# alpenlabs/dv-pari

Hardware: AMD Instinct MI355X
Metric: R1CS constraints/sec (prove) (higher is better)
Workload: dtype u32; 1 GPU; Proof::prove, synthetic dense R1CS, 2^20 constraints (BASELINE config #4); log2_constraints=20, n_wires=1048576, msm_pairs_per_proof=6291456, witness=resident in HBM, entry=dvp_prove_dev (Proof::prove with the witness resident), proofs_in_flight=1

## Files before the change

dv-pari_amd/csrc/msm_rounds.cuh:

```cuda
#pragma once
#include "common.h"
#include "k233.cuh"
#include "msm_scan.cuh"
#include "msm_reduce.cuh"

namespace dvp {

constexpr uint32_t AFF_NONE = 0xffffffffu;
constexpr uint32_t DESC_PAIR = 0x80000000u;

__global__ void __launch_bounds__(256)
k_post_sort(uint32_t* __restrict__ items, const uint32_t* __restrict__ cnt, const uint32_t* __restrict__ off , uint32_t nkeys,
            uint32_t* __restrict__ ocnt, uint32_t* __restrict__ ooff , uint32_t* __restrict__ d_max) {
  const uint32_t k = blockIdx.x * blockDim.x + threadIdx.x;
  uint32_t m = 0;
  if (k <= nkeys) {
    const uint32_t o = off[k];
    ooff[k] = o >> 1;
    if (k < nkeys) {
      const uint32_t c = cnt[k];
      if (c & 1) items[o + c] = AFF_NONE;
      ocnt[k] = (c + 1) >> 1;
      m = c;
    }
  }
  for (int o = 32; o > 0; o >>= 1) m = max(m, (uint32_t)__shfl_xor((int)m, o));
  if ((threadIdx.x & 63) == 0 && m) atomicMax(d_max, m);
}

__global__ void __launch_bounds__(SCAN_TPB) k_mscan_local(const uint32_t* __restrict__ cnt0, uint32_t m, int R, uint32_t* __restrict__ rp,
                                                          uint32_t* __restrict__ bs ) {
  __shared__ uint32_t sh[SCAN_TPB];
  const uint32_t base = blockIdx.x * SCAN_BLK + threadIdx.x * SCAN_EPT;
  uint32_t v[SCAN_EPT];
#pragma unroll
  for (int k = 0; k < SCAN_EPT; ++k) v[k] = (base + k < m) ? cnt0[base + k] : 0;
  {
    uint32_t mx = 0;
#pragma unroll
    for (int k = 0; k < SCAN_EPT; ++k) mx = max(mx, v[k]);
    for (int d = 32; d > 0; d >>= 1) mx = max(mx, (uint32_t)__shfl_xor((int)mx, d));
    if ((threadIdx.x & 63) == 0) sh[threadIdx.x >> 6] = mx;
    __syncthreads();
    if (threadIdx.x == 0) {
      for (int w = 1; w < SCAN_TPB / 64; ++w) mx = max(mx, sh[w]);
      bs[(size_t)R * gridDim.x + blockIdx.x] = mx;
    }
    __syncthreads();
  }
  for (int r = 1; r <= R; ++r) {
    uint32_t* c = rp + (size_t)(2 * (r - 1)) * ((size_t)m + 1);
    uint32_t* o = c + ((size_t)m + 1);
    uint32_t s = 0;
#pragma unroll
    for (int k = 0; k < SCAN_EPT; ++k) {
      v[k] = (v[k] + 1u) >> 1;
      s += v[k];
    }
    uint32_t tot;
    uint32_t ex = block_exclusive_scan(s, &tot, sh);
#pragma unroll
    for (int k = 0; k < SCAN_EPT; ++k) {
      if (base + k < m) {
        c[base + k] = v[k];
        o[base + k] = ex;
      }
      ex += v[k];
    }
    if (threadIdx.x == 0) bs[(size_t)(r - 1) * gridDim.x + blockIdx.x] = tot;
  }
}
__global__ void __launch_bounds__(SCAN_TPB) k_mscan_bsums(uint32_t* __restrict__ bs, uint32_t nb, uint32_t m, uint32_t* __restrict__ rp,
                                                          uint32_t* __restrict__ off0 ,
                                                          uint32_t* __restrict__ dmax ) {
  __shared__ uint32_t sh[SCAN_TPB];
  const int r = blockIdx.x + 1;
  uint32_t* row = bs + (size_t)(r - 1) * nb;
  uint32_t carry = 0;
  for (uint32_t base = 0; base < nb; base += SCAN_TPB) {
    uint32_t idx = base + threadIdx.x;
    uint32_t v = idx < nb ? row[idx] : 0;
    uint32_t tot;
    uint32_t ex = block_exclusive_scan(v, &tot, sh);
    if (idx < nb) row[idx] = ex + carry;
    carry += tot;
  }
  if (threadIdx.x == 0) {
    rp[(size_t)(2 * (r - 1) + 1) * ((size_t)m + 1) + m] = carry;
    if (r == 1 && off0) off0[m] = 2u * carry;
  }
  if (r == 1 && dmax) {
    const uint32_t* bm = bs + (size_t)gridDim.x * nb;
    uint32_t mx = 0;
    for (uint32_t i = threadIdx.x; i < nb; i += SCAN_TPB) mx = max(mx, bm[i]);
    for (int d = 32; d > 0; d >>= 1) mx = max(mx, (uint32_t)__shfl_xor((int)mx, d));
    __syncthreads();
    if ((threadIdx.x & 63) == 0) sh[threadIdx.x >> 6] = mx;
    __syncthreads();
    if (threadIdx.x == 0) {
      for (int w = 1; w < SCAN_TPB / 64; ++w) mx = max(mx, sh[w]);
      *dmax = mx;
    }
  }
}
__global__ void __launch_bounds__(SCAN_TPB) k_mscan_add(uint32_t* __restrict__ rp, const uint32_t* __restrict__ bs, uint32_t m, int R,
                                                        const uint32_t* __restrict__ cnt0, uint32_t* __restrict__ off0, uint32_t* __restrict__ items) {
  const uint32_t base = blockIdx.x * SCAN_BLK + threadIdx.x * SCAN_EPT;
  for (int r = 1; r <= R; ++r) {
    uint32_t* o = rp + (size_t)(2 * (r - 1) + 1) * ((size_t)m + 1);
    const uint32_t add = bs[(size_t)(r - 1) * gridDim.x + blockIdx.x];
    if (r == 1 && off0) {
#pragma unroll
      for (int k = 0; k < SCAN_EPT; ++k)
        if (base + k < m) {
          const uint32_t v = o[base + k] + add, c = cnt0[base + k];
          o[base + k] = v;
          off0[base + k] = 2u * v;
          if (c & 1u) items[2u * v + c] = AFF_NONE;
        }
      continue;
    }
#pragma unroll
    for (int k = 0; k < SCAN_EPT; ++k)
      if (base + k < m) o[base + k] += add;
  }
}
struct DescPlan {
  unsigned long long at[40];
};
template <int LPK, bool DENSE>
__global__ void __launch_bounds__(1024)
k_round_desc_all(const uint32_t* __restrict__ rp, uint32_t nkeys, int R, DescPlan plan, uint32_t* __restrict__ desc) {
  const uint32_t gid = blockIdx.x * blockDim.x + threadIdx.x;
  const uint32_t key = gid / LPK, lane = gid % LPK;
  if (key >= nkeys) return;
  const size_t stride = (size_t)nkeys + 1;
  for (int r0 = 1; r0 < R; r0 += 8) {
    uint32_t cr[8], o[8], oo[8], A[8];
#pragma unroll
    for (int q = 0; q < 8; ++q) {
      const int r = r0 + q;
      if (r < R) {
        const uint32_t* c = rp + (size_t)(2 * (r - 1)) * stride;
        cr[q] = c[key];
        o[q] = c[stride + key];
        oo[q] = c[3 * stride + key];
        A[q] = DENSE ? c[stride + nkeys] - c[3 * stride + nkeys] : 0u;
      } else {
        cr[q] = 0; o[q] = 0; oo[q] = 0; A[q] = 0;
      }
    }
#pragma unroll
    for (int q = 0; q < 8; ++q) {
      const int r = r0 + q;
      if (r >= R) break;
      const uint32_t nout = (cr[q] + 1) >> 1;
      uint32_t* d = desc + plan.at[r];
      if (DENSE) {
        const uint32_t npair = cr[q] >> 1, a = o[q] - oo[q];
        uint2* d2 = (uint2*)d;
        for (uint32_t j = lane; j < npair; j += LPK) d2[a + j] = make_uint2((o[q] + 2 * j) | DESC_PAIR, oo[q] + j);
        if ((cr[q] & 1u) && lane == npair % LPK) d2[A[q] + (2 * oo[q] - o[q])] = make_uint2(o[q] + cr[q] - 1, oo[q] + npair);
        continue;
      }
      for (uint32_t j = lane; j < nout; j += LPK) d[oo[q] + j] = (o[q] + 2 * j) | ((2 * j + 1 < cr[q]) ? DESC_PAIR : 0u);
    }
  }
}

template <int LPK>
__global__ void __launch_bounds__(256)
k_round_desc(const uint32_t* __restrict__ cnt, const uint32_t* __restrict__ off, const uint32_t* __restrict__ ooff ,
             uint32_t nkeys, uint32_t* __restrict__ desc) {
  const uint32_t gid = blockIdx.x * blockDim.x + threadIdx.x;
  const uint32_t key = gid / LPK, lane = gid % LPK;
  if (key >= nkeys) return;
  const uint32_t c = cnt[key], o = off[key], oo = ooff[key], nout = (c + 1) >> 1;
  for (uint32_t j = lane; j < nout; j += LPK) desc[oo + j] = (o + 2 * j) | ((2 * j + 1 < c) ? DESC_PAIR : 0u);
}

#ifndef AFF_PRIO
#define AFF_PRIO 1
#endif
#ifndef AFF_XY
#define AFF_XY 1
#endif
#ifndef AFF_NUM1
#define AFF_NUM1 1
#endif
__device__ __forceinline__ void aff_set_prio(uint32_t v) {
  switch (v % 3u) {
    case 0: __builtin_amdgcn_s_setprio(0); break;
    case 1: __builtin_amdgcn_s_setprio(1); break;
    default: __builtin_amdgcn_s_setprio(2); break;
  }
}
constexpr uint32_t AFF_BMAX = 136;
__device__ __forceinline__ uint32_t aff_slots_per_thread(uint32_t total, uint32_t cap, uint32_t bmax_bmin) {
  const uint32_t bmax = bmax_bmin & 0xffu, bmin = (bmax_bmin >> 8) & 0xffu;
  const uint32_t units = (total + cap - 1) / cap;
  const uint32_t R = (units + bmax - 1) / bmax;
  const uint32_t B = R ? (units + R - 1) / R : 1;
  return B < bmin ? bmin : B;
}
constexpr uint32_t AFF_SHARE_INV = 1u << 16;
constexpr uint32_t AFF_X_SLOT_BYTES = 2048;
constexpr uint32_t aff_exchange_bytes(uint32_t waves) { return waves == 4 ? 6 * AFF_X_SLOT_BYTES : waves == 2 ? 3 * AFF_X_SLOT_BYTES : 0; }
constexpr uint32_t AFF_INV_SPREAD = 256;
__device__ __forceinline__ void aff_x_put(uint32_t lane_addr, uint32_t slot, const Gf& v) {
  const uint32_t a = lane_addr + slot * AFF_X_SLOT_BYTES;
  gf_lds_st(a, (gf_u32x4){v.w[0], v.w[1], v.w[2], v.w[3]});
  gf_lds_st(a + 1024, (gf_u32x4){v.w[4], v.w[5], v.w[6], v.w[7]});
}
__device__ __forceinline__ Gf aff_x_get(uint32_t lane_addr, uint32_t slot) {
  const uint32_t a = lane_addr + slot * AFF_X_SLOT_BYTES;
  const gf_u32x4 lo = gf_lds_ld(a), hi = gf_lds_ld(a + 1024);
  Gf r;
  r.w[0] = lo.x; r.w[1] = lo.y; r.w[2] = lo.z; r.w[3] = lo.w;
  r.w[4] = hi.x; r.w[5] = hi.y; r.w[6] = hi.z; r.w[7] = hi.w;
  return r;
}
struct WaveTrace {
  unsigned long long* buf;
  uint32_t cap, tag;
};
struct AffSlot {
  uint32_t a, b, o;
};
template <bool FIRST, bool TRACE = false, bool DENSE = false>
__global__ void __launch_bounds__(EC_TPB) __attribute__((amdgpu_waves_per_eu(3, 3)))
k_affine_round(const Aff* __restrict__ pts, const uint2* __restrict__ desc, const uint32_t* __restrict__ total_ptr ,
               uint32_t cap, uint32_t bmax, GfSqrTables T, Gf* __restrict__ prefix, Aff* __restrict__ out, uint32_t sign_mask, WaveTrace wt) {
  extern __shared__ char lds_raw[];
  unsigned long long tr_t0 = 0, tr_c0 = 0, tr_t1 = 0, tr_t2 = 0;
  uint32_t tr_inverted = 0;
  if (TRACE) { tr_t0 = wall_clock64(); tr_c0 = clock64(); }
  GfLdsK L = gf_ldsk_init(lds_raw);
#if AFF_PRIO
  const uint32_t wslot = __builtin_amdgcn_s_getreg(((4 - 1) << 11) | 4);
#endif
  const uint32_t sm = FIRST ? sign_mask : 0u;
  auto ldx = [&](uint32_t v) -> Gf { return pts[v & ~sm].x; };
  auto ldy = [&](uint32_t v, const Gf& x) -> Gf {
    Gf y = pts[v & ~sm].y;
    if (v & sm) y = gf_add(y, x);
    return y;
  };
  const uint32_t total = *total_ptr;
  const int B = (int)aff_slots_per_thread(total, cap, bmax);
  const uint32_t nthr = (total + B - 1) / B;
  const uint32_t tid = blockIdx.x * blockDim.x + threadIdx.x;
  const bool share = (bmax & AFF_SHARE_INV) != 0 && blockDim.x > 64;
  if (share ? blockIdx.x * blockDim.x >= nthr : tid >= nthr) return;
  const bool wave_live = __builtin_amdgcn_readfirstlane(tid & ~63u) < nthr;
  const uint2 none = make_uint2(AFF_NONE, AFF_NONE);
  auto ld_desc = [&](int k) -> AffSlot {
    const uint32_t sk = (uint32_t)k * nthr + tid;
    const bool ok = k >= 0 && k < B && sk < total && tid < nthr;
    if (FIRST) {
      uint2 v = none;
      if (ok) v = desc[sk];
      return AffSlot{v.x, v.y, 0u};
    }
    const uint2 d = DENSE ? desc[ok ? sk : 0u] : make_uint2(((const uint32_t*)desc)[ok ? sk : 0u], 0u);
    const uint32_t a = d.x & ~DESC_PAIR;
    return AffSlot{ok ? a : AFF_NONE, (ok && (d.x & DESC_PAIR)) ? a + 1 : AFF_NONE, d.y};
  };
  const Gf one = gf_one();
  Gf run = one;
  if (wave_live) {
    AffSlot d0 = ld_desc(0), d1 = ld_desc(1);
    Gf xa = gf_zero(), xb = gf_zero();
    if (d0.b != AFF_NONE) { xa = ldx(d0.a); xb = ldx(d0.b); }
#if AFF_NUM1
    Gf ya = gf_zero(), yb = gf_zero();
    if (d0.b != AFF_NONE) { ya = ldy(d0.a, xa); yb = ldy(d0.b, xb); }
#endif
#pragma unroll 1
    for (int k = 0; k < B; ++k) {
#if AFF_PRIO
      aff_set_prio(wslot + (uint32_t)k);
#endif
      const AffSlot d2 = ld_desc(k + 2);
      Gf nxa = gf_zero(), nxb = gf_zero();
      if (d1.b != AFF_NONE) { nxa = ldx(d1.a); nxb = ldx(d1.b); }
#if AFF_NUM1
      Gf nya = gf_zero(), nyb = gf_zero();
      if (d1.b != AFF_NONE) { nya = ldy(d1.a, nxa); nyb = ldy(d1.b, nxb); }
#endif
      const bool pair = d0.b != AFF_NONE;
      if (!DENSE || __any(pair)) {
        Gf den = one;
#if AFF_NUM1
        Gf num = gf_zero();
        if (pair && !gf_is_zero(xa) && !gf_is_zero(xb)) {
          const Gf dd = gf_add(xa, xb), ys = gf_add(ya, yb);
          if (!gf_is_zero(dd)) { den = dd; num = ys; }
          else if (gf_is_zero(ys)) { den = xa; num = ya; }
        }
        Gf np, nrun;
        gf_mul2(num, den, run, L, np, nrun);
        if (pair) prefix[(size_t)k * nthr + tid] = np;
        run = nrun;
#else
        if (pair && !gf_is_zero(xa) && !gf_is_zero(xb)) {
          Gf dd = gf_add(xa, xb);
          if (!gf_is_zero(dd)) den = dd;
          else if (gf_eq(ldy(d0.a, xa), ldy(d0.b, xb))) den = xa;
        }
        if (pair) prefix[(size_t)k * nthr + tid] = run;
        run = gf_mul(run, den, L);
#endif
      }
      d0 = d1; d1 = d2; xa = nxa; xb = nxb;
#if AFF_NUM1
      ya = nya; yb = nyb;
#endif
    }
  }
  if (TRACE) tr_t1 = wall_clock64();
  const uint32_t W = blockDim.x >> 6, w = __builtin_amdgcn_readfirstlane(threadIdx.x >> 6);
  const uint32_t xa = L.lane_base + (W - w) * GF_LDSK_BYTES_PER_WAVE;
  const uint32_t inverting = (blockIdx.x / AFF_INV_SPREAD) & (W - 1);
  Gf inv = run;
  if (share) {
    if (TRACE) tr_inverted = w == inverting ? 3u : 2u;
    aff_x_put(xa, w, run);
    __syncthreads();
    if (W == 4) {
      if ((w & 1u) == 0) aff_x_put(xa, 4 + (w >> 1), gf_mul(run, aff_x_get(xa, w + 1), L));
      __syncthreads();
    }
    if (w == inverting) {
      __builtin_amdgcn_s_setprio(3);
      inv = gf_mul(aff_x_get(xa, W == 4 ? 4 : 0), aff_x_get(xa, W == 4 ? 5 : 1), L);
    }
  }
  if (!share || w == inverting) inv = gf_inv_fast(inv, T, L);
  if (share) {
    if (w == inverting) {
      if (W == 4) {
        Gf ia, ib;
        gf_mul2(aff_x_get(xa, 5), aff_x_get(xa, 4), inv, L, ia, ib);
        aff_x_put(xa, 4, ia);
        aff_x_put(xa, 5, ib);
      } else {
        aff_x_put(xa, 2, inv);
      }
      __builtin_amdgcn_s_setprio(0);
    }
    __syncthreads();
    inv = gf_mul(aff_x_get(xa, W == 4 ? 4 + (w >> 1) : 2), aff_x_get(xa, w ^ 1u), L);
  }
  if (TRACE) tr_t2 = wall_clock64();
  if (wave_live) {
    AffSlot e0 = ld_desc(B - 1), e1 = ld_desc(B - 2);
    Gf px = gf_zero(), qx = gf_zero(), pre = one;
    if (e0.a != AFF_NONE) px = ldx(e0.a);
    if (e0.b != AFF_NONE) { qx = ldx(e0.b); pre = prefix[(size_t)(B - 1) * nthr + tid]; }
#if AFF_XY
    Gf py = gf_zero();
    if (e0.a != AFF_NONE) py = ldy(e0.a, px);
#if !AFF_NUM1
    Gf qy = gf_zero();
    if (e0.b != AFF_NONE) qy = ldy(e0.b, qx);
#endif
#endif
#pragma unroll 1
    for (int k = B - 1; k >= 0; --k) {
#if AFF_PRIO
      aff_set_prio(wslot + (uint32_t)k);
#endif
      const AffSlot e2 = ld_desc(k - 2);
#if AFF_XY
      Gf npx = gf_zero(), nqx = gf_zero(), npy = gf_zero(), npre = one;
      if (e1.a != AFF_NONE) { npx = ldx(e1.a); npy = ldy(e1.a, npx); }
#if AFF_NUM1
      if (e1.b != AFF_NONE) { nqx = ldx(e1.b); npre = prefix[(size_t)(k - 1) * nthr + tid]; }
#else
      Gf nqy = gf_zero();
      if (e1.b != AFF_NONE) { nqx = ldx(e1.b); nqy = ldy(e1.b, nqx); npre = prefix[(size_t)(k - 1) * nthr + tid]; }
#endif
#else
      Gf py = gf_zero();
      if (e0.a != AFF_NONE) py = ldy(e0.a, px);
#if !AFF_NUM1
      Gf qy = gf_zero();
      if (e0.b != AFF_NONE) qy = ldy(e0.b, qx);
#endif
      Gf npx = gf_zero(), nqx = gf_zero(), npre = one;
      if (e1.a != AFF_NONE) npx = ldx(e1.a);
      if (e1.b != AFF_NONE) { nqx = ldx(e1.b); npre = prefix[(size_t)(k - 1) * nthr + tid]; }
#endif
#if AFF_NUM1
      auto q_y = [&]() -> Gf { return ldy(e0.b, qx); };
#else
      auto q_y = [&]() -> Gf { return qy; };
#endif
      if (e0.a != AFF_NONE) {
        const uint32_t sidx = DENSE ? e0.o : (uint32_t)k * nthr + tid;
        Gf ox = px, oy = py;
        if (e0.b != AFF_NONE) {
          if (gf_is_zero(px)) { ox = qx; oy = q_y(); }
          else if (!gf_is_zero(qx)) {
            Gf dd = gf_add(px, qx);
            const bool same_x = gf_is_zero(dd);
            const bool dbl = same_x && gf_eq(py, q_y());
            if (same_x && !dbl) {
              ox = gf_zero(); oy = gf_zero();
            } else {
              Gf den = dbl ? px : dd;
#if AFF_NUM1
              Gf lam, inv_next;
              gf_mul2(pre, den, inv, L, lam, inv_next);
              inv = inv_next;
#else
              Gf dinv, inv_next;
              gf_mul2(pre, den, inv, L, dinv, inv_next);
              inv = inv_next;
              Gf num = dbl ? py : gf_add(py, qy);
              Gf lam = gf_mul(num, dinv, L);
#endif
              if (dbl) lam = gf_add(lam, px);
              ox = gf_add(gf_add(gf_sqr(lam), lam), dd);
              oy = gf_add(gf_add(gf_mul(gf_add(px, ox), lam, L), ox), py);
            }
          }
        }
        out[sidx].x = ox; out[sidx].y = oy;
      }
      e0 = e1; e1 = e2; px = npx; qx = nqx; pre = npre;
#if AFF_XY
      py = npy;
#if !AFF_NUM1
      qy = nqy;
#endif
#endif
    }
  }
#if AFF_PRIO
  __builtin_amdgcn_s_setprio(0);
#endif
  if (TRACE) {
    const unsigned long long t3 = wall_clock64(), c3 = clock64();
    if ((threadIdx.x & 63u) == 0) {
      const unsigned long long i = atomicAdd(wt.buf, 1ull);
      if (i < wt.cap) {
        unsigned long long* r = wt.buf + 8 + 8 * i;
        r[0] = tr_t0; r[1] = tr_t1; r[2] = tr_t2; r[3] = t3;
        r[4] = tr_c0; r[5] = c3;
        r[6] = (unsigned long long)__builtin_amdgcn_s_getreg((31 << 11) | 4) | ((unsigned long long)__builtin_amdgcn_s_getreg((31 << 11) | 20) << 32);
        r[7] = (unsigned long long)blockIdx.x | ((unsigned long long)wt.tag << 32) | ((unsigned long long)(uint32_t)B << 48) | ((unsigned long long)(threadIdx.x >> 6) << 56) |
               ((unsigned long long)tr_inverted << 60);
      }
    }
  }
}

__global__ void __launch_bounds__(256)
k_bucket_gather_aff(const Aff* __restrict__ in, const uint32_t* __restrict__ cnt, const uint32_t* __restrict__ off,
                    uint32_t nkeys, Ld* __restrict__ A) {
  uint32_t k = blockIdx.x * blockDim.x + threadIdx.x;
  if (k >= nkeys) return;
  Ld r = ld_infinity();
  if (cnt[k]) {
    Aff p = in[off[k]];
    if (!gf_is_zero(p.x)) r = ld_from_aff(p);
  }
  A[k] = r;
}
__global__ void __launch_bounds__(256)
k_bucket_gather_items(const Aff* __restrict__ bases, const uint32_t* __restrict__ items, const uint32_t* __restrict__ cnt,
                      const uint32_t* __restrict__ off, uint32_t nkeys, Ld* __restrict__ A, uint32_t sign_mask) {
  uint32_t k = blockIdx.x * blockDim.x + threadIdx.x;
  if (k >= nkeys) return;
  Ld r = ld_infinity();
  if (cnt[k]) {
    const uint32_t v = items[off[k]];
    Aff q = bases[v & ~sign_mask];
    if (v & sign_mask) q.y = gf_add(q.y, q.x);
    r = ld_from_aff(q);
  }
  A[k] = r;
}

__global__ void __launch_bounds__(256)
k_bucket_gather(const Ld* __restrict__ in, const uint32_t* __restrict__ cnt, const uint32_t* __restrict__ off,
                uint32_t nkeys, Ld* __restrict__ A) {
  uint32_t k = blockIdx.x * blockDim.x + threadIdx.x;
  if (k >= nkeys) return;
  A[k] = cnt[k] ? in[off[k]] : ld_infinity();
}

}
```

Measured before the change: 59.17 million constraints/s.

## Flag rare affine-add cases in prefix words and load points branch-free

Rewrites the batched-affine addition kernel so the forward pass computes den and num unconditionally. It detects infinity, same-x and doubling cases with OR-reduction, and encodes the rare outcome in spare high bits of the stored prefix product. The backward pass reads those flags instead of re-checking zero/equality and reloading q's y, and only leaves the common add path when a flag is set. Point and descriptor loads become unconditional (index 0 when absent), the sign fix-up becomes a mask-xor, and slot indices advance by addition instead of multiplication. The intent is to cut divergent branches, redundant y loads and extra comparisons. In exchange it issues extra loads for empty slots and depends on the top bits of word 7 being unused by K-233 field elements.

```diff
diff --git a/dv-pari_amd/csrc/msm_rounds.cuh b/dv-pari_amd/csrc/msm_rounds.cuh
--- a/dv-pari_amd/csrc/msm_rounds.cuh
+++ b/dv-pari_amd/csrc/msm_rounds.cuh
@@ -182,12 +182,10 @@
 #ifndef AFF_PRIO
 #define AFF_PRIO 1
 #endif
-#ifndef AFF_XY
-#define AFF_XY 1
-#endif
-#ifndef AFF_NUM1
-#define AFF_NUM1 1
-#endif
+constexpr uint32_t AFF_W7_MASK = 0x1ffu, AFF_W7_DBL = 1u << 30, AFF_W7_SKIP = 1u << 31;
+__device__ __forceinline__ uint32_t aff_or8(const Gf& a) {
+  return ((a.w[0] | a.w[1] | a.w[2]) | (a.w[3] | a.w[4])) | ((a.w[5] | a.w[6]) | a.w[7]);
+}
 __device__ __forceinline__ void aff_set_prio(uint32_t v) {
   switch (v % 3u) {
     case 0: __builtin_amdgcn_s_setprio(0); break;
@@ -227,6 +225,26 @@
 struct AffSlot {
   uint32_t a, b, o;
 };
+template <bool FIRST>
+__device__ __forceinline__ void aff_ld_point(const Aff* __restrict__ pts, uint32_t sm, uint32_t v, Gf& x, Gf& y) {
+  const Aff* p = pts + (v & ~sm);
+  x = p->x;
+  y = p->y;
+  if (FIRST) {
+    const uint32_t neg = 0u - (uint32_t)((v & sm) != 0u);
+#pragma unroll
+    for (int i = 0; i < 8; ++i) y.w[i] = gf_andxor(neg, x.w[i], y.w[i]);
+  }
+}
+template <bool FIRST, bool DENSE>
+__device__ __forceinline__ AffSlot aff_ld_desc(const uint2* __restrict__ desc, int k, int B, uint32_t sk, uint32_t lim) {
+  const bool ok = k >= 0 && k < B && sk < lim;
+  const uint32_t at = ok ? sk : 0u;
+  const uint2 d = (FIRST || DENSE) ? desc[at] : make_uint2(((const uint32_t*)desc)[at], 0u);
+  if (FIRST) return AffSlot{ok ? d.x : AFF_NONE, ok ? d.y : AFF_NONE, 0u};
+  const uint32_t a = d.x & ~DESC_PAIR;
+  return AffSlot{ok ? a : AFF_NONE, (ok && (d.x & DESC_PAIR)) ? a + 1 : AFF_NONE, d.y};
+}
 template <bool FIRST, bool TRACE = false, bool DENSE = false>
 __global__ void __launch_bounds__(EC_TPB) __attribute__((amdgpu_waves_per_eu(3, 3)))
 k_affine_round(const Aff* __restrict__ pts, const uint2* __restrict__ desc, const uint32_t* __restrict__ total_ptr ,
@@ -241,11 +259,7 @@
 #endif
   const uint32_t sm = FIRST ? sign_mask : 0u;
   auto ldx = [&](uint32_t v) -> Gf { return pts[v & ~sm].x; };
-  auto ldy = [&](uint32_t v, const Gf& x) -> Gf {
-    Gf y = pts[v & ~sm].y;
-    if (v & sm) y = gf_add(y, x);
-    return y;
-  };
+  auto ldp = [&](uint32_t v, Gf& x, Gf& y) { aff_ld_point<FIRST>(pts, sm, v, x, y); };
   const uint32_t total = *total_ptr;
   const int B = (int)aff_slots_per_thread(total, cap, bmax);
   const uint32_t nthr = (total + B - 1) / B;
@@ -253,69 +267,61 @@
   const bool share = (bmax & AFF_SHARE_INV) != 0 && blockDim.x > 64;
   if (share ? blockIdx.x * blockDim.x >= nthr : tid >= nthr) return;
   const bool wave_live = __builtin_amdgcn_readfirstlane(tid & ~63u) < nthr;
-  const uint2 none = make_uint2(AFF_NONE, AFF_NONE);
-  auto ld_desc = [&](int k) -> AffSlot {
-    const uint32_t sk = (uint32_t)k * nthr + tid;
-    const bool ok = k >= 0 && k < B && sk < total && tid < nthr;
-    if (FIRST) {
-      uint2 v = none;
-      if (ok) v = desc[sk];
-      return AffSlot{v.x, v.y, 0u};
-    }
-    const uint2 d = DENSE ? desc[ok ? sk : 0u] : make_uint2(((const uint32_t*)desc)[ok ? sk : 0u], 0u);
-    const uint32_t a = d.x & ~DESC_PAIR;
-    return AffSlot{ok ? a : AFF_NONE, (ok && (d.x & DESC_PAIR)) ? a + 1 : AFF_NONE, d.y};
-  };
+  const uint32_t lim = tid < nthr ? total : 0u;
+  auto ld_desc = [&](int k, uint32_t sk) -> AffSlot { return aff_ld_desc<FIRST, DENSE>(desc, k, B, sk, lim); };
   const Gf one = gf_one();
   Gf run = one;
   if (wave_live) {
-    AffSlot d0 = ld_desc(0), d1 = ld_desc(1);
-    Gf xa = gf_zero(), xb = gf_zero();
-    if (d0.b != AFF_NONE) { xa = ldx(d0.a); xb = ldx(d0.b); }
-#if AFF_NUM1
-    Gf ya = gf_zero(), yb = gf_zero();
-    if (d0.b != AFF_NONE) { ya = ldy(d0.a, xa); yb = ldy(d0.b, xb); }
-#endif
+    uint32_t sk = tid, sp = tid;
+    AffSlot d0 = ld_desc(0, sk);
+    sk += nthr;
+    AffSlot d1 = ld_desc(1, sk);
+    sk += nthr;
+    Gf xa, ya, xb, yb;
+    {
+      const bool p = d0.b != AFF_NONE;
+      ldp(p ? d0.a : 0u, xa, ya);
+      ldp(p ? d0.b : 0u, xb, yb);
+    }
 #pragma unroll 1
     for (int k = 0; k < B; ++k) {
 #if AFF_PRIO
       aff_set_prio(wslot + (uint32_t)k);
 #endif
-      const AffSlot d2 = ld_desc(k + 2);
-      Gf nxa = gf_zero(), nxb = gf_zero();
-      if (d1.b != AFF_NONE) { nxa = ldx(d1.a); nxb = ldx(d1.b); }
-#if AFF_NUM1
-      Gf nya = gf_zero(), nyb = gf_zero();
-      if (d1.b != AFF_NONE) { nya = ldy(d1.a, nxa); nyb = ldy(d1.b, nxb); }
-#endif
       const bool pair = d0.b != AFF_NONE;
+      Gf den = gf_add(xa, xb), num = gf_add(ya, yb);
+      const bool ainf = aff_or8(xa) == 0u, binf = aff_or8(xb) == 0u;
+      const bool rare = pair & (ainf | binf | (aff_or8(den) == 0u));
+      bool dbl = false;
+      den.w[0] |= pair ? 0u : 1u;
+      if (__any(rare)) {
+        if (rare) {
+          dbl = !ainf & !binf & (aff_or8(num) == 0u);
+          den = dbl ? xa : one;
+          num = dbl ? ya : gf_zero();
+        }
+      }
+      const AffSlot d2 = ld_desc(k + 2, sk);
+      sk += nthr;
+      {
+        const bool p = d1.b != AFF_NONE;
+        if (!DENSE || __any(p)) {
+          ldp(p ? d1.a : 0u, xa, ya);
+          ldp(p ? d1.b : 0u, xb, yb);
+        }
+      }
       if (!DENSE || __any(pair)) {
-        Gf den = one;
-#if AFF_NUM1
-        Gf num = gf_zero();
-        if (pair && !gf_is_zero(xa) && !gf_is_zero(xb)) {
-          const Gf dd = gf_add(xa, xb), ys = gf_add(ya, yb);
-          if (!gf_is_zero(dd)) { den = dd; num = ys; }
-          else if (gf_is_zero(ys)) { den = xa; num = ya; }
-        }
         Gf np, nrun;
         gf_mul2(num, den, run, L, np, nrun);
-        if (pair) prefix[(size_t)k * nthr + tid] = np;
+        if (__any(rare)) {
+          if (rare) np.w[7] |= dbl ? AFF_W7_DBL : AFF_W7_SKIP;
+        }
+        if (pair) prefix[sp] = np;
         run = nrun;
-#else
-        if (pair && !gf_is_zero(xa) && !gf_is_zero(xb)) {
-          Gf dd = gf_add(xa, xb);
-          if (!gf_is_zero(dd)) den = dd;
-          else if (gf_eq(ldy(d0.a, xa), ldy(d0.b, xb))) den = xa;
-        }
-        if (pair) prefix[(size_t)k * nthr + tid] = run;
-        run = gf_mul(run, den, L);
-#endif
-      }
-      d0 = d1; d1 = d2; xa = nxa; xb = nxb;
-#if AFF_NUM1
-      ya = nya; yb = nyb;
-#endif
+      }
+      sp += nthr;
+      d0 = d1;
+      d1 = d2;
     }
   }
   if (TRACE) tr_t1 = wall_clock64();
@@ -354,88 +360,72 @@
   }
   if (TRACE) tr_t2 = wall_clock64();
   if (wave_live) {
-    AffSlot e0 = ld_desc(B - 1), e1 = ld_desc(B - 2);
-    Gf px = gf_zero(), qx = gf_zero(), pre = one;
-    if (e0.a != AFF_NONE) px = ldx(e0.a);
-    if (e0.b != AFF_NONE) { qx = ldx(e0.b); pre = prefix[(size_t)(B - 1) * nthr + tid]; }
-#if AFF_XY
-    Gf py = gf_zero();
-    if (e0.a != AFF_NONE) py = ldy(e0.a, px);
-#if !AFF_NUM1
-    Gf qy = gf_zero();
-    if (e0.b != AFF_NONE) qy = ldy(e0.b, qx);
-#endif
-#endif
+    uint32_t sp = (uint32_t)(B - 1) * nthr + tid, sk = sp;
+    auto ld_slot = [&](const AffSlot& e, uint32_t s, Gf& x1, Gf& y1, Gf& x2, Gf& pre) {
+      const bool pair = e.b != AFF_NONE;
+      ldp(e.a != AFF_NONE ? e.a : 0u, x1, y1);
+      x2 = ldx(pair ? e.b : 0u);
+      pre = prefix[pair ? s : 0u];
+    };
+    AffSlot e0 = ld_desc(B - 1, sk);
+    sk -= nthr;
+    AffSlot e1 = ld_desc(B - 2, sk);
+    sk -= nthr;
+    Gf px, py, qx, pre;
+    ld_slot(e0, sp, px, py, qx, pre);
 #pragma unroll 1
     for (int k = B - 1; k >= 0; --k) {
 #if AFF_PRIO
       aff_set_prio(wslot + (uint32_t)k);
 #endif
-      const AffSlot e2 = ld_desc(k - 2);
-#if AFF_XY
-      Gf npx = gf_zero(), nqx = gf_zero(), npy = gf_zero(), npre = one;
-      if (e1.a != AFF_NONE) { npx = ldx(e1.a); npy = ldy(e1.a, npx); }
-#if AFF_NUM1
-      if (e1.b != AFF_NONE) { nqx = ldx(e1.b); npre = prefix[(size_t)(k - 1) * nthr + tid]; }
-#else
-      Gf nqy = gf_zero();
-      if (e1.b != AFF_NONE) { nqx = ldx(e1.b); nqy = ldy(e1.b, nqx); npre = prefix[(size_t)(k - 1) * nthr + tid]; }
-#endif
-#else
-      Gf py = gf_zero();
-      if (e0.a != AFF_NONE) py = ldy(e0.a, px);
-#if !AFF_NUM1
-      Gf qy = gf_zero();
-      if (e0.b != AFF_NONE) qy = ldy(e0.b, qx);
-#endif
-      Gf npx = gf_zero(), nqx = gf_zero(), npre = one;
-      if (e1.a != AFF_NONE) npx = ldx(e1.a);
-      if (e1.b != AFF_NONE) { nqx = ldx(e1.b); npre = prefix[(size_t)(k - 1) * nthr + tid]; }
-#endif
-#if AFF_NUM1
-      auto q_y = [&]() -> Gf { return ldy(e0.b, qx); };
-#else
-      auto q_y = [&]() -> Gf { return qy; };
-#endif
-      if (e0.a != AFF_NONE) {
-        const uint32_t sidx = DENSE ? e0.o : (uint32_t)k * nthr + tid;
-        Gf ox = px, oy = py;
-        if (e0.b != AFF_NONE) {
-          if (gf_is_zero(px)) { ox = qx; oy = q_y(); }
-          else if (!gf_is_zero(qx)) {
-            Gf dd = gf_add(px, qx);
-            const bool same_x = gf_is_zero(dd);
-            const bool dbl = same_x && gf_eq(py, q_y());
-            if (same_x && !dbl) {
-              ox = gf_zero(); oy = gf_zero();
-            } else {
-              Gf den = dbl ? px : dd;
-#if AFF_NUM1
-              Gf lam, inv_next;
-              gf_mul2(pre, den, inv, L, lam, inv_next);
-              inv = inv_next;
-#else
-              Gf dinv, inv_next;
-              gf_mul2(pre, den, inv, L, dinv, inv_next);
-              inv = inv_next;
-              Gf num = dbl ? py : gf_add(py, qy);
-              Gf lam = gf_mul(num, dinv, L);
-#endif
-              if (dbl) lam = gf_add(lam, px);
-              ox = gf_add(gf_add(gf_sqr(lam), lam), dd);
-              oy = gf_add(gf_add(gf_mul(gf_add(px, ox), lam, L), ox), py);
-            }
+      const bool pair = e0.b != AFF_NONE, flagged = pair & (pre.w[7] > AFF_W7_MASK);
+      const uint32_t sidx = DENSE ? e0.o : sp;
+      Gf dd = gf_add(px, qx);
+      bool add = pair, dbl = false;
+      if (__any(flagged)) {
+        if (flagged) {
+          dbl = (pre.w[7] & AFF_W7_DBL) != 0u;
+          if (dbl) {
+            pre.w[7] &= AFF_W7_MASK;
+            dd = px;
+          } else {
+            add = false;
+            const bool pinf = aff_or8(px) == 0u, qinf = aff_or8(qx) == 0u;
+            Gf qy, unused;
+            ldp(e0.b, unused, qy);
+            out[sidx].x = pinf ? qx : qinf ? px : gf_zero();
+            out[sidx].y = pinf ? qy : qinf ? py : gf_zero();
           }
         }
-        out[sidx].x = ox; out[sidx].y = oy;
-      }
-      e0 = e1; e1 = e2; px = npx; qx = nqx; pre = npre;
-#if AFF_XY
+      }
+      const AffSlot e2 = ld_desc(k - 2, sk);
+      sk -= nthr;
+      Gf npx, npy, npre;
+      ld_slot(e1, sp - nthr, npx, npy, qx, npre);
+      if (add) {
+        Gf lam, inv_next;
+        gf_mul2(pre, dd, inv, L, lam, inv_next);
+        inv = inv_next;
+        if (__any(dbl)) {
+          if (dbl) {
+            lam = gf_add(lam, px);
+            dd = gf_zero();
+          }
+        }
+        const Gf ox = gf_add(gf_add(gf_sqr(lam), lam), dd);
+        const Gf oy = gf_add(gf_add(gf_mul(gf_add(px, ox), lam, L), ox), py);
+        out[sidx].x = ox;
+        out[sidx].y = oy;
+      } else if (e0.a != AFF_NONE && !pair) {
+        out[sidx].x = px;
+        out[sidx].y = py;
+      }
+      sp -= nthr;
+      e0 = e1;
+      e1 = e2;
+      px = npx;
       py = npy;
-#if !AFF_NUM1
-      qy = nqy;
-#endif
-#endif
+      pre = npre;
     }
   }
 #if AFF_PRIO
```

Result: faster. 60.55 million constraints/s (median of 6 runs) (+2.3%).
